# travistangvh/time-series-kafka-demo

Hardware: AMD Instinct MI355X
Metric: waveform_windows_per_sec (higher is better)
Workload: dtype bf16; 1 GPU; model=MyCNN5, global_batch=65536, seq_len=120, streams_per_gpu=65536, fs_hz=125, hipgraph=True, overlap=False, parallelism=dp1, mode=pipeline

## Files before the change

### tskd_amd/engine/stream_engine.py

```python

from __future__ import annotations

import ctypes
from typing import Optional, Sequence

import numpy as np
import os

import torch

from tskd_amd.engine import windowing as W

_plib: Optional[ctypes.CDLL] = None


def _load_preproc_lib() -> ctypes.CDLL:
    global _plib
    if _plib is not None:
        return _plib
    import os

    from tskd_amd.ops import build as _build
    path = _build.lib_path("_tskd_preprocess")
    if not os.path.exists(path):
# ... 110 lines not shown
        if chan_map is None:
            chan_map = list(range(cin))
        if self._gpu:
            lib = _load_preproc_lib()
            raw = raw.contiguous()
            is_bf16 = 1 if raw.dtype == torch.bfloat16 else 0
            if not is_bf16 and raw.dtype != torch.float32:
                raw = raw.float()
            key = tuple(chan_map)
            cm = getattr(self, "_cm_cache", {}).get(key)
            if cm is None:
                cm = torch.tensor(list(chan_map), dtype=torch.int32,
                                  device=self.device)
                self._cm_cache = getattr(self, "_cm_cache", {})
                self._cm_cache[key] = cm
            rc = lib.tskd_preproc_ingest_dense(
                ctypes.c_void_p(raw.data_ptr()), is_bf16,
                ctypes.c_void_p(self.bsum.data_ptr()),
                ctypes.c_void_p(self.bcnt.data_ptr()),
                ctypes.c_void_p(cm.data_ptr()),
                self.S, cin, self.C, t, self.G, self.bucket_len,
                ctypes.c_long(self.head), self._dstate_ptr(), self._bst,
                _sptr())
            if rc != 0:
                raise RuntimeError(f"ingest_dense failed: hipError {rc}")
            self._clear_stale_channels(chan_map, nb)
        else:
            rawf = raw.float().cpu().numpy()
            for j in range(nb):
                seg = rawf[:, :, j * self.bucket_len:(j + 1) * self.bucket_len]
                ok = ~np.isnan(seg)
                g = (self.head + j) % self.G
                for ci, c in enumerate(chan_map):
                    self.bsum[:, c, g] = torch.from_numpy(
                        np.where(ok[:, ci], seg[:, ci], 0.0).sum(-1)).float()
                    self.bcnt[:, c, g] = torch.from_numpy(
                        ok[:, ci].sum(-1).astype(np.float64)).float()
                other = [c for c in range(self.C) if c not in chan_map]
                if other:
                    self.bsum[:, other, g] = 0
                    self.bcnt[:, other, g] = 0
        self.head += nb
        self._cleared = max(self._cleared, self.head)
        self._refill()
        return nb

    def _clear_stale_channels(self, chan_map: Sequence[int], nb: int) -> None:
        other = [c for c in range(self.C) if c not in set(chan_map)]
        if not other or nb <= 0:
            return
        idx = torch.tensor([(self.head + j) % self.G for j in range(nb)],
                           dtype=torch.long, device=self.device)
        oth = torch.tensor(other, dtype=torch.long, device=self.device)
        self.bsum[:, oth[:, None], idx[None, :]] = 0
        self.bcnt[:, oth[:, None], idx[None, :]] = 0

    def ingest_events(self, stream_idx: torch.Tensor, chan_idx: torch.Tensor,
                      ts: torch.Tensor, vals: torch.Tensor,
                      advance_to: Optional[float] = None) -> None:
        if len(ts) == 0 and advance_to is None:
            return
        if (len(ts) and self.head == 0 and self.nproc == 0
                and self._origin_nproc == 0):
            first_bucket = int(float(ts.min()) // self.bucket_s)
            if first_bucket > self.G:
                self._origin_nproc = first_bucket
        min_bucket = self.nproc
        if self._gpu:
            tsd = ts.double().to(self.device) if not ts.is_cuda else ts.double()
            bucket_d = torch.floor(tsd / self.bucket_s).long()
            if len(bucket_d):
                bmax = int(bucket_d.max().item())
                bmin = int(bucket_d.min().item())
                if bmax - max(bmin, min_bucket) >= self.G - self.win_buckets:
                    raise ValueError(
                        "event batch spans more buckets than the ring "
                        "holds; ingest in smaller chunks")
                self._clear_ahead(bmax + 1)
            else:
                self._clear_ahead(0)
            lib = _load_preproc_lib()
            si = stream_idx.to(torch.int32).contiguous().to(self.device)
            ci = chan_idx.to(torch.int32).contiguous().to(self.device)
            bi = bucket_d.contiguous()
            vi = vals.float().contiguous().to(self.device)
            rc = lib.tskd_preproc_ingest_events(
                ctypes.c_void_p(si.data_ptr()), ctypes.c_void_p(ci.data_ptr()),
                ctypes.c_void_p(bi.data_ptr()), ctypes.c_void_p(vi.data_ptr()),
                ctypes.c_void_p(self.bsum.data_ptr()),
                ctypes.c_void_p(self.bcnt.data_ptr()),
                self.C, self.G, ctypes.c_long(len(vi)),
                ctypes.c_long(min_bucket), self._bst, _sptr())
            if rc != 0:
                raise RuntimeError(f"ingest_events failed: hipError {rc}")
            if advance_to is None and len(tsd):
                advance_to = float(tsd.max().item())
        else:
            bucket = torch.floor(ts.double() / self.bucket_s).long()
            if len(bucket) and int(bucket.max()) - max(int(bucket.min()),
                                                       min_bucket) \
                    >= self.G - self.win_buckets:
                raise ValueError("event batch spans more buckets than the "
                                 "ring holds; ingest in smaller chunks")
            self._clear_ahead(int(bucket.max().item()) + 1 if len(bucket)
                              else 0)
            ok = (~torch.isnan(vals)) & (bucket >= min_bucket)
            if ok.any():
                flat = ((stream_idx[ok].numpy() * self.C
                         + chan_idx[ok].numpy()) * self.G
                        + (bucket[ok].numpy() % self.G))
                bs = self.bsum.numpy().reshape(-1)
                bc = self.bcnt.numpy().reshape(-1)
                np.add.at(bs, flat, vals[ok].numpy().astype(np.float64))
                np.add.at(bc, flat, 1.0)
        hwm = float(advance_to) if advance_to is not None else float(ts.max())
        new_head = int(np.floor(hwm / self.bucket_s))
        if new_head > self.head:
            self.head = new_head
        self._refill()

    def ingest_events_chunked(self, stream_idx, chan_idx, ts, vals,
                              advance_to=None) -> None:
        cap = self.G - self.win_buckets - 1
        if len(ts) == 0:
            if advance_to is not None:
                self.ingest_events(stream_idx, chan_idx, ts, vals,
                                   advance_to=advance_to)
            return
        bucket = torch.floor(ts.double() / self.bucket_s).long()
        span = int(bucket.max()) - max(int(bucket.min()), self.nproc)
        if span < cap:
            self.ingest_events(stream_idx, chan_idx, ts, vals,
                               advance_to=advance_to)
            return
        order = torch.argsort(bucket)
        b_sorted = bucket[order]
        lo = 0
        n = len(order)
        while lo < n:
            start_bucket = max(int(b_sorted[lo]), self.nproc)
            hi = int(torch.searchsorted(b_sorted,
                                        torch.tensor(start_bucket + cap)))
            hi = max(hi, lo + 1)
            idx = order[lo:hi]
            chunk_adv = float((int(b_sorted[min(hi, n) - 1]) + 1)
                              * self.bucket_s)
            self.ingest_events(stream_idx[idx], chan_idx[idx], ts[idx],
                               vals[idx], advance_to=chunk_adv)
            lo = hi
        if advance_to is not None and advance_to / self.bucket_s > self.head:
            self._clear_ahead(int(advance_to / self.bucket_s))
            self.head = int(advance_to / self.bucket_s)
            self._refill()

    def _clear_ahead(self, upto_bucket: int) -> None:
        if upto_bucket <= self._cleared:
            return
        start = max(self._cleared, upto_bucket - self.G)
        nb = upto_bucket - start
        if self._gpu:
            lib = _load_preproc_lib()
            rc = lib.tskd_preproc_clear_buckets(
                ctypes.c_void_p(self.bsum.data_ptr()),
                ctypes.c_void_p(self.bcnt.data_ptr()),
                self.S, self.C, self.G, ctypes.c_long(start), nb,
                self._bst, _sptr())
            if rc != 0:
                raise RuntimeError(f"clear_buckets failed: hipError {rc}")
        else:
            idx = np.arange(start, start + nb) % self.G
            self.bsum[:, :, idx] = 0
            self.bcnt[:, :, idx] = 0
        self._cleared = upto_bucket

    def ingest_graph_kernel(self, raw: torch.Tensor, chan_map) -> None:
        lib = _load_preproc_lib()
        cin, t = raw.shape[1], raw.shape[2]
        key = tuple(chan_map)
        cm = getattr(self, "_cm_cache", {}).get(key)
        if cm is None:
            cm = torch.tensor(list(chan_map), dtype=torch.int32,
                              device=self.device)
            self._cm_cache = getattr(self, "_cm_cache", {})
            self._cm_cache[key] = cm
        is_bf16 = 1 if raw.dtype == torch.bfloat16 else 0
        rc = lib.tskd_preproc_ingest_dense(
            ctypes.c_void_p(raw.data_ptr()), is_bf16,
            ctypes.c_void_p(self.bsum.data_ptr()),
            ctypes.c_void_p(self.bcnt.data_ptr()),
            ctypes.c_void_p(cm.data_ptr()),
            self.S, cin, self.C, t, self.G, self.bucket_len,
            ctypes.c_long(0), self._dstate_ptr(), self._bst, _sptr())
        if rc != 0:
            raise RuntimeError(f"ingest(graph) failed: {rc}")

    def fill_graph_kernel(self, nb: int) -> None:
        lib = _load_preproc_lib()
        rc = lib.tskd_preproc_window_fill(
            ctypes.c_void_p(self.bsum.data_ptr()),
            ctypes.c_void_p(self.bcnt.data_ptr()),
            ctypes.c_void_p(self.proc.data_ptr()),
            ctypes.c_void_p(self.last_val.data_ptr()),
            self.S, self.C, self.G, ctypes.c_long(0), nb,
            self.win_buckets, self._dstate_ptr(), self._bst, _sptr())
        if rc != 0:
            raise RuntimeError(f"fill(graph) failed: {rc}")

    def ingest_dense_graph_body(self, raw: torch.Tensor, chan_map, nb: int
                                 ) -> None:
        self.ingest_graph_kernel(raw, chan_map)
        self.fill_graph_kernel(nb)

    def _refill(self) -> None:
        navail = max(0, self.head - self.win_buckets + 1)
        np_new = navail - self.nproc
        if np_new <= 0:
            return
        max_np = self.G - self.win_buckets
        if np_new > max_np:
            self.nproc = navail - max_np
            np_new = max_np
        if self._gpu:
            lib = _load_preproc_lib()
            rc = lib.tskd_preproc_window_fill(
                ctypes.c_void_p(self.bsum.data_ptr()),
                ctypes.c_void_p(self.bcnt.data_ptr()),
                ctypes.c_void_p(self.proc.data_ptr()),
                ctypes.c_void_p(self.last_val.data_ptr()),
                self.S, self.C, self.G, ctypes.c_long(self.nproc), np_new,
                self.win_buckets, self._dstate_ptr(), self._bst, _sptr())
            if rc != 0:
                raise RuntimeError(f"window_fill failed: hipError {rc}")
        else:
            bs = self.bsum.numpy()
            bc = self.bcnt.numpy()
            pr = self.proc.numpy()
            lv = self.last_val.numpy()
            span = np_new + self.win_buckets - 1
            gidx = (self.nproc + np.arange(span)) % self.G
            pidx = (self.nproc + np.arange(np_new)) % self.G
            for s in range(self.S):
                for c in range(self.C):
                    vals = W.window_averages(bs[s, c, gidx], bc[s, c, gidx],
                                             self.win_buckets)
                    filled, carry = W.fill_series(vals, lv[s, c])
                    pr[s, c, pidx] = filled
                    lv[s, c] = carry
        self.nproc = navail

    def windows(self, batch: int = 1, stride: int = 12,
                dtype: torch.dtype = torch.float32,
                out: Optional[torch.Tensor] = None,
                timelast: bool = False,
                znormalize: bool = False, zeps: float = 1e-6) -> torch.Tensor:
        B, WIN = batch, self.model_win
        assert (B - 1) * stride + WIN <= self.G, (
            f"windows(batch={B}, stride={stride}) reaches back "
            f"{(B - 1) * stride + WIN} grid points but the ring holds only "
            f"G={self.G} — older slots are already overwritten")
        shape = (self.S, B, WIN, self.C) if timelast \
            else (self.S, B, self.C, WIN)
        provided = out is not None
        if out is not None:
            assert out.shape == shape and out.dtype == dtype
            assert out.is_contiguous()
        out = out if out is not None else torch.zeros(
            shape, dtype=dtype, device=self.device)
        if self._gpu:
            lib = _load_preproc_lib()
            is_bf16 = 1 if dtype == torch.bfloat16 else 0
            assert dtype in (torch.bfloat16, torch.float32)
            rc = lib.tskd_preproc_window_gather(
                ctypes.c_void_p(self.proc.data_ptr()),
                ctypes.c_void_p(out.data_ptr()), is_bf16, int(timelast),
                self.S, self.C, self.G, B, WIN, stride,
                ctypes.c_long(self.nproc), self._dstate_ptr(),
                self._dstate_gather_extra, _sptr())
            if rc == 0 and znormalize:
                assert not timelast, "znormalize needs channel-major windows"
                rc = lib.tskd_preproc_window_znorm(
                    ctypes.c_void_p(out.data_ptr()), is_bf16,
                    ctypes.c_long(self.S * B * self.C), WIN,
                    ctypes.c_float(zeps), _sptr())
            if rc != 0:
                raise RuntimeError(f"window_gather failed: hipError {rc}")
        else:
            pr = self.proc.numpy()
            if provided:
                out.zero_()
            for b in range(B):
                wend = self.nproc - (B - 1 - b) * stride
                if wend - WIN < 0:
                    continue
                idx = (np.arange(wend - WIN, wend)) % self.G
                w = torch.from_numpy(pr[:, :, idx]).to(dtype)
                out[:, b] = w.transpose(-1, -2) if timelast else w
            if znormalize:
                assert not timelast
                m = out.float().mean(dim=-1, keepdim=True)
                sd = out.float().std(dim=-1, unbiased=False, keepdim=True)
                out.copy_(((out.float() - m) / sd.clamp_min(zeps)).to(dtype))
        return out

    @property
    def ready(self) -> bool:
        return getattr(self, "_forced_ready", False) or \
            self.nproc - self._origin_nproc >= self.model_win

    def force_ready(self) -> None:
        self._forced_ready = True


class TriggerGraph:

    def __init__(self, engine: "StreamEngine", raw: torch.Tensor,
                 chan_map, graphed_forward, stride: int = 12,
                 overlap: bool = False):
        assert engine._gpu, "TriggerGraph needs a CUDA StreamEngine"
        cin, t = raw.shape[1], raw.shape[2]
        self.nb = t // engine.bucket_len
        assert engine.nproc == engine.head - engine.win_buckets + 1, \
            "engine must be in steady state (warm up with eager triggers)"
        self.engine = engine
        self.raw = raw.contiguous()
        self.gf = graphed_forward
        self.stride = stride
        self.chan_map = list(chan_map)
        self.overlap = overlap
        dev = engine.device
        self.dstate = torch.tensor([engine.head, engine.nproc],
                                   dtype=torch.int64, device=dev)
        lib = _load_preproc_lib()
        self._lib = lib
        if overlap:
            self._init_overlap()
            return

        def trigger_body():
            engine._dstate = self.dstate
            engine._dstate_gather_extra = self.nb
            try:
                engine.ingest_dense_graph_body(self.raw, self.chan_map,
                                               self.nb)
                engine.windows(batch=1, stride=stride, dtype=self.gf.x.dtype,
                               out=self.gf.x,
                               timelast=getattr(self.gf, "timelast", False))
                out = self.gf.engine.forward(self.gf.x, self.gf.age,
                                             apply_sigmoid=True)
                rc = lib.tskd_preproc_advance_state(
                    ctypes.c_void_p(self.dstate.data_ptr()), self.nb,
                    self.nb, _sptr())
                if rc != 0:
                    raise RuntimeError(f"advance_state: {rc}")
                return out
            finally:
                engine._dstate = None
                engine._dstate_gather_extra = 0

        stream = torch.cuda.Stream()
        with torch.cuda.stream(stream):
            trigger_body()
        torch.cuda.current_stream().wait_stream(stream)
        engine.head += self.nb
        engine.nproc += self.nb
        self.graph = torch.cuda.CUDAGraph()
        with torch.cuda.graph(self.graph):
            self.out = trigger_body()

    def _init_overlap(self) -> None:
        engine, lib = self.engine, self._lib
        nb = self.nb

        def ingest_body():
            engine._dstate = self.dstate
            try:
                engine.ingest_graph_kernel(self.raw, self.chan_map)
                rc = lib.tskd_preproc_advance_state(
                    ctypes.c_void_p(self.dstate.data_ptr()), nb, 0, _sptr())
                if rc != 0:
                    raise RuntimeError(f"advance_state(head): {rc}")
            finally:
                engine._dstate = None

        def model_body():
            engine._dstate = self.dstate
            engine._dstate_gather_extra = nb
            try:
                engine.fill_graph_kernel(nb)
                engine.windows(batch=1, stride=self.stride,
                               dtype=self.gf.x.dtype, out=self.gf.x,
                               timelast=getattr(self.gf, "timelast", False))
                out = self.gf.engine.forward(self.gf.x, self.gf.age,
                                             apply_sigmoid=True)
                rc = lib.tskd_preproc_advance_state(
                    ctypes.c_void_p(self.dstate.data_ptr()), 0, nb, _sptr())
                if rc != 0:
                    raise RuntimeError(f"advance_state(nproc): {rc}")
                return out
            finally:
                engine._dstate = None
                engine._dstate_gather_extra = 0

        self._sA = torch.cuda.Stream()
        self._sB = torch.cuda.Stream()
        with torch.cuda.stream(self._sA):
            ingest_body()
        self._sB.wait_stream(self._sA)
        with torch.cuda.stream(self._sB):
            model_body()
        torch.cuda.current_stream().wait_stream(self._sB)
        engine.head += nb
        engine.nproc += nb
        self.graph_i = torch.cuda.CUDAGraph()
        with torch.cuda.graph(self.graph_i, stream=self._sA):
            ingest_body()
        self.graph_m = torch.cuda.CUDAGraph()
        with torch.cuda.graph(self.graph_m, stream=self._sB):
            self.out = model_body()
        self._evA = torch.cuda.Event()

    def replay(self, raw_refresh: bool = False) -> torch.Tensor:
        if self.overlap:
            cur = torch.cuda.current_stream()
            if raw_refresh:
                self._sA.wait_stream(cur)
            with torch.cuda.stream(self._sA):
                self.graph_i.replay()
                self._evA.record(self._sA)
            self._sB.wait_event(self._evA)
            self._sB.wait_stream(cur)
            with torch.cuda.stream(self._sB):
                self.graph_m.replay()
            cur.wait_stream(self._sB)
            self.engine.head += self.nb
            self.engine.nproc += self.nb
            return self.out
        self.graph.replay()
        self.engine.head += self.nb
        self.engine.nproc += self.nb
        return self.out
```

### tskd_amd/ops/__init__.py

```python

from __future__ import annotations

import ctypes
import os
from typing import Optional

import torch

from tskd_amd.ops import build as _build
from tskd_amd.ops.pack import (VARIANT_IDS, pack_conv1_mfma_bfrags,
                               pack_weights)

_lib: Optional[ctypes.CDLL] = None
_lib_err: Optional[str] = None


def _load_lib() -> ctypes.CDLL:
    global _lib, _lib_err
    if _lib is not None:
        return _lib
    path = _build.lib_path("_tskd_mycnn")
    if not os.path.exists(path):
        try:
            _build.build("_tskd_mycnn")
        except Exception as e:
            _lib_err = f"hipcc build failed: {e}"
            raise RuntimeError(_lib_err)
    lib = ctypes.CDLL(path)
    lib.tskd_conv_fwd.restype = ctypes.c_int
    lib.tskd_conv_fwd.argtypes = [
        ctypes.c_void_p, ctypes.c_int, ctypes.c_int, ctypes.c_void_p,
        ctypes.c_void_p, ctypes.c_void_p, ctypes.c_int, ctypes.c_int,
        ctypes.c_void_p,
    ]
    lib.tskd_debug_mfma16x16x32.restype = ctypes.c_int
    lib.tskd_debug_mfma16x16x32.argtypes = [
        ctypes.c_void_p, ctypes.c_void_p, ctypes.c_void_p, ctypes.c_void_p,
    ]
    lib.tskd_lstm_head_fwd.restype = ctypes.c_int
    lib.tskd_lstm_head_fwd.argtypes = [
        ctypes.c_void_p, ctypes.c_void_p, ctypes.c_void_p, ctypes.c_void_p,
        ctypes.c_int, ctypes.c_int, ctypes.c_float, ctypes.c_int,
        ctypes.c_int, ctypes.c_void_p,
    ]
    lib.tskd_pack_size.restype = ctypes.c_int
    lib.tskd_pack_size.argtypes = [ctypes.c_int]
    lib.tskd_feat_len.restype = ctypes.c_int
    lib.tskd_feat_len.argtypes = [ctypes.c_int]
    _lib = lib
    return lib


def hip_available() -> bool:
    try:
        _load_lib()
        return True
    except Exception:
        return False


def _stream_ptr() -> ctypes.c_void_p:
    return ctypes.c_void_p(torch.cuda.current_stream().cuda_stream)


TLAST_SLACK = 256


def alloc_windows(s: int, n: int, cin: int, win: int = 120,
                  timelast: bool = False, dtype=torch.bfloat16,
                  device="cuda") -> torch.Tensor:
    numel = s * n * cin * win
    buf = torch.zeros(numel + TLAST_SLACK, dtype=dtype, device=device)
    shape = (s, n, win, cin) if timelast else (s, n, cin, win)
    t = buf[:numel].view(*shape)
    t._tskd_slack = True
    t._tskd_buf = buf
    return t


class MyCNNEngine:

    def __init__(self, model, device: str = "cuda"):
        from tskd_amd.models.mycnn import _MyCNNBase
        assert isinstance(model, _MyCNNBase)
        self.variant = VARIANT_IDS[type(model).__name__]
        self.age_eps = float(model.AGE_EPS)
        self.cin = int(model.IN_CHANNELS)
        self.device = torch.device(device)
        self.model = model
        self.wpack = pack_weights(model).to(self.device)
        self.bfrag = pack_conv1_mfma_bfrags(model).to(self.device)
        if self.device.type == "cuda":
            lib = _load_lib()
            expect = lib.tskd_pack_size(self.variant)
            if expect != self.wpack.numel():
                raise RuntimeError(
                    f"weight pack size mismatch: py={self.wpack.numel()} "
                    f"hip={expect}")
            self.feat_len = lib.tskd_feat_len(self.variant)
        else:
            self.feat_len = int(model.MAGICNUM)

    def conv_features(self, x: torch.Tensor) -> torch.Tensor:
        timelast = (x.shape[-1] == self.cin and x.shape[-2] == 120
                    and self.cin != 120)
        lead = x.shape[:-2]
        xf = x.reshape(-1, x.shape[-2], x.shape[-1]).contiguous()
        sn = xf.shape[0]
        if xf.device.type != "cuda":
            raise RuntimeError("conv_features is the GPU path; use the model on CPU")
        lib = _load_lib()
        if timelast and (self.cin % 2 != 0 or xf.dtype != torch.bfloat16):
            xf = xf.transpose(-1, -2).contiguous()
            timelast = False
        if xf.dtype == torch.bfloat16:
            is_bf16 = 1
        elif xf.dtype == torch.float32:
            is_bf16 = 0
        else:
            xf = xf.to(torch.float32)
            is_bf16 = 0
        if timelast and not getattr(x, "_tskd_slack", False):
            pad = alloc_windows(1, sn, self.cin, 120, timelast=True,
                                dtype=xf.dtype, device=xf.device)
            pad.reshape(-1).copy_(xf.reshape(-1))
            xf = pad.reshape(sn, 120, self.cin)
        feat = torch.empty(sn, self.feat_len, dtype=torch.float32, device=xf.device)
        rc = lib.tskd_conv_fwd(
            ctypes.c_void_p(xf.data_ptr()), is_bf16, int(timelast),
            ctypes.c_void_p(feat.data_ptr()),
            ctypes.c_void_p(self.wpack.data_ptr()),
            ctypes.c_void_p(self.bfrag.data_ptr()), sn, self.variant,
            _stream_ptr())
        if rc != 0:
            raise RuntimeError(f"tskd_conv_fwd failed: hipError {rc}")
        return feat.reshape(*lead, self.feat_len)

    def lstm_head(self, feat: torch.Tensor, age: Optional[torch.Tensor],
                  apply_sigmoid: bool = False) -> torch.Tensor:
        assert feat.dim() == 3 and feat.shape[-1] == self.feat_len
        s, n = feat.shape[0], feat.shape[1]
        feat = feat.contiguous()
        lib = _load_lib()
        out = torch.empty(s, n, dtype=torch.float32, device=feat.device)
        age_ptr = ctypes.c_void_p(0)
        if age is not None:
            if age.dtype != torch.float32 or age.shape != (s, n) \
                    or not age.is_contiguous():
                age = age.to(torch.float32).expand(s, n).contiguous()
            age_ptr = ctypes.c_void_p(age.data_ptr())
        rc = lib.tskd_lstm_head_fwd(
            ctypes.c_void_p(feat.data_ptr()), age_ptr,
            ctypes.c_void_p(out.data_ptr()),
            ctypes.c_void_p(self.wpack.data_ptr()), s, n,
            ctypes.c_float(self.age_eps), int(apply_sigmoid), self.variant,
            _stream_ptr())
        if rc != 0:
            raise RuntimeError(f"tskd_lstm_head_fwd failed: hipError {rc}")
        return out

    def forward(self, x: torch.Tensor, age: Optional[torch.Tensor] = None,
                apply_sigmoid: bool = False) -> torch.Tensor:
        squeeze = x.dim() == 3
        if squeeze:
            x = x.unsqueeze(0)
            if age is not None and age.dim() == 1:
                age = age.unsqueeze(0)
        assert x.dim() == 4 and (
            (x.shape[-1] == 120 and x.shape[-2] == self.cin)
            or (x.shape[-2] == 120 and x.shape[-1] == self.cin))
        if x.device.type == "cuda":
            s, n = x.shape[0], x.shape[1]
            feat = self.conv_features(x).reshape(s, n, self.feat_len)
            out = self.lstm_head(feat, age, apply_sigmoid)
        else:
            s, n = x.shape[0], x.shape[1]
            if x.shape[-1] == self.cin and x.shape[-2] == 120:
                x = x.transpose(-1, -2)
            with torch.no_grad():
                outs = []
                for i in range(s):
                    a = age[i] if age is not None else torch.zeros(n)
                    y = self.model(x[i].float(), a.float())
                    outs.append(torch.sigmoid(y) if apply_sigmoid else y)
                out = torch.stack(outs)
        return out[0] if squeeze else out

    __call__ = forward


class GraphedForward:

    def __init__(self, engine: "MyCNNEngine", s: int, n: int,
                 dtype: torch.dtype = torch.bfloat16,
                 apply_sigmoid: bool = True, warmup: int = 2,
                 timelast: bool = False, capture: bool = True):
        assert engine.device.type == "cuda"
        self.engine = engine
        self.timelast = timelast
        self.x = alloc_windows(s, n, engine.cin, 120, timelast=timelast,
                               dtype=dtype, device=engine.device)
        self.age = torch.full((s, n), 65.0, device=engine.device)
        self.graph = None
        if not capture:
            return
        stream = torch.cuda.Stream()
        with torch.cuda.stream(stream):
            for _ in range(warmup):
                out = engine.forward(self.x, self.age,
                                     apply_sigmoid=apply_sigmoid)
        torch.cuda.current_stream().wait_stream(stream)
        self.graph = torch.cuda.CUDAGraph()
        with torch.cuda.graph(self.graph):
            self.out = engine.forward(self.x, self.age,
                                      apply_sigmoid=apply_sigmoid)

    def replay(self) -> torch.Tensor:
        self.graph.replay()
        return self.out
```

### tskd_amd/ops/csrc/mycnn_kernels.hip

```cpp

#include <hip/hip_runtime.h>
#include <stdlib.h>

#define WAVE 64
#define WG_WAVES 4
#define WG_THREADS (WAVE * WG_WAVES)

typedef __attribute__((ext_vector_type(8))) __bf16 bf16x8;
typedef __attribute__((ext_vector_type(4))) float f32x4;

template <int CIN_, int K1_, int PK_, int PS_, int L_ = 120>
struct Geom {
    static constexpr int CIN = CIN_;
    static constexpr int K1  = K1_;
    static constexpr int PK  = PK_;
    static constexpr int PS  = PS_;
    static constexpr int L   = L_;
    static constexpr int C1  = L - K1 + 1;
    static constexpr int P1  = (C1 - PK) / PS + 1;
    static constexpr int C2  = P1 - 5 + 1;
    static constexpr int LIN = (C2 - PK) / PS + 1;
    static constexpr int KK     = CIN * K1;
    static constexpr int KSTEPS = (KK + 31) / 32;
    static constexpr int MTILES = (C1 + 15) / 16;
// ... 231 lines not shown
    constexpr int NW = 4 * G::CIN * G::K1 + 4 + 20 + 1;
    __shared__ float lds_w[NW];
    __shared__ float lds_c1[WG_WAVES][4 * G::C1];
    __shared__ float lds_p1[WG_WAVES][4 * G::P1];
    __shared__ float lds_c2[WG_WAVES][G::C2];

    for (int i = threadIdx.x; i < NW; i += WG_THREADS) lds_w[i] = wpack[i];
    __syncthreads();

    const int wave = threadIdx.x / WAVE;
    const int lane = threadIdx.x % WAVE;
    const float* b1 = lds_w + G::OB1;

    bf16x8 bfr[G::KSTEPS];
    union BU { unsigned int d[4]; unsigned short u[8]; bf16x8 v; };
    #pragma unroll
    for (int st = 0; st < G::KSTEPS; ++st) {
        BU bu;
        #pragma unroll
        for (int q = 0; q < 4; ++q)
            bu.d[q] = ((const unsigned int*)bfrag)[(st * WAVE + lane) * 4 + q];
        bfr[st] = bu.v;
    }
    const int lane_dw = ((lane & 15) * G::CIN + (lane >> 4) * 8) / 2;
    __shared__ float lds_c1b[WG_WAVES][4 * G::C1];

    for (long win = (blockIdx.x * WG_WAVES + wave) * 2; win < SN;
         win += (long)gridDim.x * WG_WAVES * 2) {
        const long win1 = win + 1;
        const bool has1 = win1 < SN;
        const unsigned int* xwa =
            (const unsigned int*)(x + win * (long)(G::L * G::CIN));
        const unsigned int* xwb =
            (const unsigned int*)(x + (has1 ? win1 : win) *
                                  (long)(G::L * G::CIN));
        #pragma unroll 1
        for (int mt = 0; mt < G::MTILES; ++mt) {
            f32x4 acca = {0.f, 0.f, 0.f, 0.f};
            f32x4 accb = {0.f, 0.f, 0.f, 0.f};
            const unsigned int* basea = xwa + (long)mt * (16 * G::CIN / 2)
                                        + lane_dw;
            const unsigned int* baseb = xwb + (long)mt * (16 * G::CIN / 2)
                                        + lane_dw;
            #pragma unroll
            for (int st = 0; st < G::KSTEPS; ++st) {
                BU aa, ab;
                aa.d[0] = basea[st * 16 + 0];
                aa.d[1] = basea[st * 16 + 1];
                aa.d[2] = basea[st * 16 + 2];
                aa.d[3] = basea[st * 16 + 3];
                ab.d[0] = baseb[st * 16 + 0];
                ab.d[1] = baseb[st * 16 + 1];
                ab.d[2] = baseb[st * 16 + 2];
                ab.d[3] = baseb[st * 16 + 3];
                acca = __builtin_amdgcn_mfma_f32_16x16x32_bf16(aa.v, bfr[st],
                                                               acca, 0, 0, 0);
                accb = __builtin_amdgcn_mfma_f32_16x16x32_bf16(ab.v, bfr[st],
                                                               accb, 0, 0, 0);
            }
            const int c = lane & 15;
            if (c < 4) {
                #pragma unroll
                for (int r = 0; r < 4; ++r) {
                    const int row = mt * 16 + (lane >> 4) * 4 + r;
                    if (row < G::C1) {
                        lds_c1[wave][c * G::C1 + row] = acca[r] + b1[c];
                        lds_c1b[wave][c * G::C1 + row] = accb[r] + b1[c];
                    }
                }
            }
        }
        wave_sync();
        conv_tail<G, true>(lane, lds_w, lds_c1[wave], lds_p1[wave],
                           lds_c2[wave], feat, win);
        if (has1)
            conv_tail<G, true>(lane, lds_w, lds_c1b[wave], lds_p1[wave],
                               lds_c2[wave], feat, win1);
    }
}

template <class G>
__global__ __launch_bounds__(WG_THREADS) void conv_stack_mfma_wg_kernel(
    const unsigned short* __restrict__ x,
    float* __restrict__ feat,
    const float* __restrict__ wpack,
    const unsigned short* __restrict__ bfrag,
    int SN)
{
    constexpr int NW = 4 * G::CIN * G::K1 + 4 + 20 + 1;
    __shared__ float lds_w[NW];
    __shared__ float lds_c1[4 * G::C1];
    __shared__ float lds_p1[4 * G::P1];
    __shared__ float lds_c2[G::C2];

    for (int i = threadIdx.x; i < NW; i += WG_THREADS) lds_w[i] = wpack[i];
    __syncthreads();

    const int wave = threadIdx.x / WAVE;
    const int lane = threadIdx.x % WAVE;
    const float* b1 = lds_w + G::OB1;
    const float* w2 = lds_w + G::OW2;
    const float b2 = lds_w[G::OB2];

    bf16x8 bfr[G::KSTEPS];
    union BU { unsigned int d[4]; unsigned short u[8]; bf16x8 v; };
    #pragma unroll
    for (int st = 0; st < G::KSTEPS; ++st) {
        BU bu;
        #pragma unroll
        for (int q = 0; q < 4; ++q)
            bu.d[q] = ((const unsigned int*)bfrag)[(st * WAVE + lane) * 4 + q];
        bfr[st] = bu.v;
    }
    const int lane_dw = ((lane & 15) * G::CIN + (lane >> 4) * 8) / 2;

    for (long win = blockIdx.x; win < SN; win += gridDim.x) {
        const unsigned int* xw =
            (const unsigned int*)(x + win * (long)(G::L * G::CIN));
        for (int mt = wave; mt < G::MTILES; mt += WG_WAVES) {
            f32x4 acc = {0.f, 0.f, 0.f, 0.f};
            const unsigned int* base = xw + (long)mt * (16 * G::CIN / 2)
                                       + lane_dw;
            #pragma unroll
            for (int st = 0; st < G::KSTEPS; ++st) {
                BU au;
                au.d[0] = base[st * 16 + 0];
                au.d[1] = base[st * 16 + 1];
                au.d[2] = base[st * 16 + 2];
                au.d[3] = base[st * 16 + 3];
                acc = __builtin_amdgcn_mfma_f32_16x16x32_bf16(au.v, bfr[st],
                                                              acc, 0, 0, 0);
            }
            const int c = lane & 15;
            if (c < 4) {
                #pragma unroll
                for (int r = 0; r < 4; ++r) {
                    const int row = mt * 16 + (lane >> 4) * 4 + r;
                    if (row < G::C1)
                        lds_c1[c * G::C1 + row] = acc[r] + b1[c];
                }
            }
        }
        __syncthreads();
        for (int o = threadIdx.x; o < 4 * G::P1; o += WG_THREADS) {
            const int c = o / G::P1, q = o % G::P1;
            const float* src = lds_c1 + c * G::C1 + q * G::PS;
            float m = src[0];
            #pragma unroll
            for (int k = 1; k < G::PK; ++k) m = fmaxf(m, src[k]);
            lds_p1[o] = tanhf_(m);
        }
        __syncthreads();
        for (int s = threadIdx.x; s < G::C2; s += WG_THREADS) {
            float acc = b2;
            #pragma unroll
            for (int c = 0; c < 4; ++c) {
                const float* pr = lds_p1 + c * G::P1 + s;
                #pragma unroll
                for (int k = 0; k < 5; ++k)
                    acc = fmaf(w2[c * 5 + k], pr[k], acc);
            }
            lds_c2[s] = acc;
        }
        __syncthreads();
        for (int q = threadIdx.x; q < G::LIN; q += WG_THREADS) {
            const float* src = lds_c2 + q * G::PS;
            float m = src[0];
            #pragma unroll
            for (int k = 1; k < G::PK; ++k) m = fmaxf(m, src[k]);
            feat[win * G::LIN + q] = tanhf_(m);
        }
        __syncthreads();
    }
}

template <class G, int CHUNK = 32>
__global__ __launch_bounds__(WG_THREADS) void lstm_head_kernel(
    const float* __restrict__ feat,
    const float* __restrict__ age,
    float* __restrict__ out,
    const float* __restrict__ wpack,
    int S, int N, float age_eps, int apply_sigmoid)
{
    constexpr int LIN = G::LIN;
    constexpr int PRE_R = (CHUNK * LIN + WAVE - 1) / WAVE;
    __shared__ float lds_feat[WG_WAVES][CHUNK * LIN];

    const int wave = threadIdx.x / WAVE;
    const int lane = threadIdx.x % WAVE;
    const int unit = lane & 15;

    float wih1[LIN], whh1[16], wih2[16], whh2[16];
    const float bl1 = wpack[G::OBL1 + lane];
    const float bl2 = wpack[G::OBL2 + lane];
    #pragma unroll
    for (int i = 0; i < LIN; ++i) wih1[i] = wpack[G::OWIH1 + lane * LIN + i];
    #pragma unroll
    for (int i = 0; i < 16; ++i) {
        whh1[i] = wpack[G::OWHH1 + lane * 16 + i];
        wih2[i] = wpack[G::OWIH2 + lane * 16 + i];
        whh2[i] = wpack[G::OWHH2 + lane * 16 + i];
    }
    const float outw = wpack[G::OOUTW + unit];
    const float outb = wpack[G::OOUTB];
    const bool is_cell_gate = (lane >= 32 && lane < 48);

    float* fw = lds_feat[wave];

    for (long seq = blockIdx.x * WG_WAVES + wave; seq < S;
         seq += (long)gridDim.x * WG_WAVES) {
        const float* fseq = feat + seq * (long)N * LIN;
        const float* aseq = age ? age + seq * N : nullptr;
        float h1v[16], h2v[16];
        float c1 = 0.f, c2 = 0.f;
        #pragma unroll
        for (int u = 0; u < 16; ++u) h1v[u] = h2v[u] = 0.f;

        const long ntot = (long)N * LIN;
        float pre[PRE_R];
        #pragma unroll
        for (int r = 0; r < PRE_R; ++r) {
            const long idx = (long)r * WAVE + lane;
            pre[r] = idx < ntot ? fseq[idx] : 0.f;
        }
        for (int t0 = 0; t0 < N; t0 += CHUNK) {
            const int tn = min(CHUNK, N - t0);
            #pragma unroll
            for (int r = 0; r < PRE_R; ++r) {
                const int j = r * WAVE + lane;
                if (j < CHUNK * LIN) fw[j] = pre[r];
            }
            wave_sync();
            if (t0 + CHUNK < N) {
                const long base = (long)(t0 + CHUNK) * LIN;
                #pragma unroll
                for (int r = 0; r < PRE_R; ++r) {
                    const long idx = base + (long)r * WAVE + lane;
                    pre[r] = idx < ntot ? fseq[idx] : 0.f;
                }
            }

            for (int tt = 0; tt < tn; ++tt) {
                const float* xt = fw + tt * LIN;
                float ga = bl1, gb = 0.f;
                #pragma unroll
                for (int i = 0; i < LIN; i += 2) {
                    ga = fmaf(wih1[i], xt[i], ga);
                    if (i + 1 < LIN) gb = fmaf(wih1[i + 1], xt[i + 1], gb);
                }
                #pragma unroll
                for (int u = 0; u < 16; u += 2) {
                    ga = fmaf(whh1[u], h1v[u], ga);
                    gb = fmaf(whh1[u + 1], h1v[u + 1], gb);
                }
                float g = ga + gb;
                float a = is_cell_gate ? tanhf_(g) : sigmoidf_(g);
                {
                    const float iu = __shfl(a, unit);
                    const float fu = __shfl(a, unit + 16);
                    const float gu = __shfl(a, unit + 32);
                    const float ou = __shfl(a, unit + 48);
                    c1 = fmaf(fu, c1, iu * gu);
                    const float h = ou * tanhf_(c1);
                    #pragma unroll
                    for (int u = 0; u < 16; ++u) h1v[u] = __shfl(h, u);
                }
                ga = bl2; gb = 0.f;
                #pragma unroll
                for (int u = 0; u < 16; u += 2) {
                    ga = fmaf(wih2[u], h1v[u], ga);
                    gb = fmaf(wih2[u + 1], h1v[u + 1], gb);
                    ga = fmaf(whh2[u], h2v[u], ga);
                    gb = fmaf(whh2[u + 1], h2v[u + 1], gb);
                }
                g = ga + gb;
                a = is_cell_gate ? tanhf_(g) : sigmoidf_(g);
                {
                    const float iu = __shfl(a, unit);
                    const float fu = __shfl(a, unit + 16);
                    const float gu = __shfl(a, unit + 32);
                    const float ou = __shfl(a, unit + 48);
                    c2 = fmaf(fu, c2, iu * gu);
                    const float h = ou * tanhf_(c2);
                    #pragma unroll
                    for (int u = 0; u < 16; ++u) h2v[u] = __shfl(h, u);
                }
                if (lane == 0) {
                    float y = outb;
                    #pragma unroll
                    for (int u = 0; u < 16; ++u)
                        y = fmaf(wpack[G::OOUTW + u], h2v[u], y);
                    const float ag = aseq ? aseq[t0 + tt] : 0.f;
                    y *= fmaxf(fmaf(ag, age_eps, 1.0f), 0.0f);
                    if (apply_sigmoid) y = sigmoidf_(y);
                    out[seq * N + t0 + tt] = y;
                }
            }
            wave_sync();
        }
    }
    (void)outw;
}

__global__ void debug_mfma_kernel(const unsigned short* __restrict__ A,
                                  const unsigned short* __restrict__ B,
                                  float* __restrict__ C) {
    const int lane = threadIdx.x;
    union BU { unsigned short u[8]; bf16x8 v; } a, b;
    #pragma unroll
    for (int j = 0; j < 8; ++j) {
        const int k = (lane >> 4) * 8 + j;
        a.u[j] = A[(lane & 15) * 32 + k];
        b.u[j] = B[k * 16 + (lane & 15)];
    }
    f32x4 acc = {0.f, 0.f, 0.f, 0.f};
    acc = __builtin_amdgcn_mfma_f32_16x16x32_bf16(a.v, b.v, acc, 0, 0, 0);
    #pragma unroll
    for (int r = 0; r < 4; ++r)
        C[((lane >> 4) * 4 + r) * 16 + (lane & 15)] = acc[r];
}

namespace {

template <class G>
int launch_conv(const void* x, int x_is_bf16, int x_timelast, float* feat,
                const float* wpack, const void* bfrag, int SN,
                hipStream_t stream) {
    if (SN <= 0) return 0;
    int grid = (SN + WG_WAVES - 1) / WG_WAVES;
    if (grid > 8192) grid = 8192;
    if (x_is_bf16) {
        if (!bfrag) return -2;
        if (x_timelast) {
            if constexpr (G::CIN % 2 == 0) {
                int onewave = 1;
                if (const char* e = getenv("TSKD_CONV_TLAST_1WAVE"))
                    onewave = atoi(e);
                if (onewave) {
                    int g1 = (SN / 2 + WG_WAVES - 1) / WG_WAVES;
                    if (g1 < 1) g1 = 1;
                    if (g1 > 8192) g1 = 8192;
                    hipLaunchKernelGGL((conv_stack_mfma_tlast_kernel<G>),
                                       dim3(g1), dim3(WG_THREADS), 0, stream,
                                       (const unsigned short*)x, feat, wpack,
                                       (const unsigned short*)bfrag, SN);
                } else {
                    int g2 = SN > 16384 ? 16384 : SN;
                    hipLaunchKernelGGL((conv_stack_mfma_wg_kernel<G>),
                                       dim3(g2), dim3(WG_THREADS), 0, stream,
                                       (const unsigned short*)x, feat, wpack,
                                       (const unsigned short*)bfrag, SN);
                }
                return (int)hipGetLastError();
            }
            return -4;
        }
        hipLaunchKernelGGL((conv_stack_mfma_kernel<G>), dim3(grid),
                           dim3(WG_THREADS), 0, stream,
                           (const unsigned short*)x, feat, wpack,
                           (const unsigned short*)bfrag, SN);
    } else {
        if (x_timelast) return -4;
        hipLaunchKernelGGL((conv_stack_kernel<G>), dim3(grid),
                           dim3(WG_THREADS), 0, stream, (const float*)x, feat,
                           wpack, SN);
    }
    return (int)hipGetLastError();
}

template <class G>
int launch_lstm(const float* feat, const float* age, float* out,
                const float* wpack, int S, int N, float age_eps,
                int apply_sigmoid, hipStream_t stream) {
    if (S <= 0 || N <= 0) return 0;
    int grid = (S + WG_WAVES - 1) / WG_WAVES;
    if (grid > 8192) grid = 8192;
    int chunk = 32;
    if (const char* e = getenv("TSKD_LSTM_CHUNK")) chunk = atoi(e);
    if (chunk >= 64)
        hipLaunchKernelGGL((lstm_head_kernel<G, 64>), dim3(grid),
                           dim3(WG_THREADS), 0, stream, feat, age, out,
                           wpack, S, N, age_eps, apply_sigmoid);
    else
        hipLaunchKernelGGL((lstm_head_kernel<G, 32>), dim3(grid),
                           dim3(WG_THREADS), 0, stream, feat, age, out,
                           wpack, S, N, age_eps, apply_sigmoid);
    return (int)hipGetLastError();
}

}

extern "C" {

int tskd_conv_fwd(const void* x, int x_is_bf16, int x_timelast, float* feat,
                  const float* wpack, const void* bfrag, int SN, int variant,
                  void* stream) {
    hipStream_t s = (hipStream_t)stream;
    switch (variant) {
        case 0: return launch_conv<GeomCNN5>(x, x_is_bf16, x_timelast, feat,
                                             wpack, bfrag, SN, s);
        case 1: return launch_conv<GeomCNN2>(x, x_is_bf16, x_timelast, feat,
                                             wpack, bfrag, SN, s);
        case 2: return launch_conv<GeomCNN4>(x, x_is_bf16, x_timelast, feat,
                                             wpack, bfrag, SN, s);
    }
    return -1;
}

int tskd_lstm_head_fwd(const float* feat, const float* age, float* out,
                       const float* wpack, int S, int N, float age_eps,
                       int apply_sigmoid, int variant, void* stream) {
    hipStream_t s = (hipStream_t)stream;
    switch (variant) {
        case 0: return launch_lstm<GeomCNN5>(feat, age, out, wpack, S, N,
                                             age_eps, apply_sigmoid, s);
        case 1: return launch_lstm<GeomCNN2>(feat, age, out, wpack, S, N,
                                             age_eps, apply_sigmoid, s);
        case 2: return launch_lstm<GeomCNN4>(feat, age, out, wpack, S, N,
                                             age_eps, apply_sigmoid, s);
    }
    return -1;
}

int tskd_debug_mfma16x16x32(const unsigned short* A, const unsigned short* B,
                            float* C, void* stream) {
    hipLaunchKernelGGL(debug_mfma_kernel, dim3(1), dim3(WAVE), 0,
                       (hipStream_t)stream, A, B, C);
    return (int)hipGetLastError();
}

int tskd_pack_size(int variant) {
    switch (variant) {
        case 0: return GeomCNN5::NPACK;
        case 1: return GeomCNN2::NPACK;
        case 2: return GeomCNN4::NPACK;
    }
    return -1;
}

int tskd_feat_len(int variant) {
    switch (variant) {
        case 0: return GeomCNN5::LIN;
        case 1: return GeomCNN2::LIN;
        case 2: return GeomCNN4::LIN;
    }
    return -1;
}

int tskd_conv_ksteps(int variant) {
    switch (variant) {
        case 0: return GeomCNN5::KSTEPS;
        case 1: return GeomCNN2::KSTEPS;
        case 2: return GeomCNN4::KSTEPS;
    }
    return -1;
}

}
```

Baseline: 35.85 million windows/s.

## Fuse ring-buffer window gather, conv and LSTM head into one serve kernel

Adds a serve_tail kernel that reads the latest 120-sample window straight from the fp32 ring buffer, converts it to bf16 in LDS, and runs the MFMA conv, conv tail and LSTM head in a single launch, two windows per wave. It replaces the separate windows() gather into a bf16 staging tensor, the conv kernel writing features to global memory, and the LSTM head kernel inside the graphed trigger. This removes intermediate global round trips and kernel launches. It costs more LDS and registers per wave and only applies under the env-gated conditions of bf16, timelast, batch 1, even channel count and window 120.

```diff
diff --git a/tskd_amd/engine/stream_engine.py b/tskd_amd/engine/stream_engine.py
--- a/tskd_amd/engine/stream_engine.py
+++ b/tskd_amd/engine/stream_engine.py
@@ -436,6 +436,13 @@
                 out.copy_(((out.float() - m) / sd.clamp_min(zeps)).to(dtype))
         return out
 
+    def score_latest(self, model_engine, age: Optional[torch.Tensor] = None,
+                     apply_sigmoid: bool = True) -> torch.Tensor:
+        assert self._gpu and self.model_win == 120
+        return model_engine.score_ring(
+            self.proc, self.G, self.nproc, self._dstate_ptr(),
+            self._dstate_gather_extra, age, apply_sigmoid)
+
     @property
     def ready(self) -> bool:
         return getattr(self, "_forced_ready", False) or \
@@ -461,6 +468,13 @@
         self.stride = stride
         self.chan_map = list(chan_map)
         self.overlap = overlap
+        gf = graphed_forward
+        self.fused_tail = (
+            os.environ.get("TSKD_FUSED_TAIL", "1") != "0"
+            and gf.x.dtype == torch.bfloat16
+            and getattr(gf, "timelast", False) and gf.x.shape[1] == 1
+            and engine.model_win == 120
+            and gf.engine.supports_fused_tail(engine.C))
         dev = engine.device
         self.dstate = torch.tensor([engine.head, engine.nproc],
                                    dtype=torch.int64, device=dev)
@@ -476,11 +490,7 @@
             try:
                 engine.ingest_dense_graph_body(self.raw, self.chan_map,
                                                self.nb)
-                engine.windows(batch=1, stride=stride, dtype=self.gf.x.dtype,
-                               out=self.gf.x,
-                               timelast=getattr(self.gf, "timelast", False))
-                out = self.gf.engine.forward(self.gf.x, self.gf.age,
-                                             apply_sigmoid=True)
+                out = self._score()
                 rc = lib.tskd_preproc_advance_state(
                     ctypes.c_void_p(self.dstate.data_ptr()), self.nb,
                     self.nb, _sptr())
@@ -500,6 +510,16 @@
         self.graph = torch.cuda.CUDAGraph()
         with torch.cuda.graph(self.graph):
             self.out = trigger_body()
+
+    def _score(self) -> torch.Tensor:
+        gf = self.gf
+        if self.fused_tail:
+            return self.engine.score_latest(gf.engine, gf.age,
+                                            apply_sigmoid=True)
+        self.engine.windows(batch=1, stride=self.stride, dtype=gf.x.dtype,
+                            out=gf.x,
+                            timelast=getattr(gf, "timelast", False))
+        return gf.engine.forward(gf.x, gf.age, apply_sigmoid=True)
 
     def _init_overlap(self) -> None:
         engine, lib = self.engine, self._lib
@@ -521,11 +541,7 @@
             engine._dstate_gather_extra = nb
             try:
                 engine.fill_graph_kernel(nb)
-                engine.windows(batch=1, stride=self.stride,
-                               dtype=self.gf.x.dtype, out=self.gf.x,
-                               timelast=getattr(self.gf, "timelast", False))
-                out = self.gf.engine.forward(self.gf.x, self.gf.age,
-                                             apply_sigmoid=True)
+                out = self._score()
                 rc = lib.tskd_preproc_advance_state(
                     ctypes.c_void_p(self.dstate.data_ptr()), 0, nb, _sptr())
                 if rc != 0:
diff --git a/tskd_amd/ops/__init__.py b/tskd_amd/ops/__init__.py
--- a/tskd_amd/ops/__init__.py
+++ b/tskd_amd/ops/__init__.py
@@ -42,6 +42,13 @@
         ctypes.c_void_p, ctypes.c_void_p, ctypes.c_void_p, ctypes.c_void_p,
         ctypes.c_int, ctypes.c_int, ctypes.c_float, ctypes.c_int,
         ctypes.c_int, ctypes.c_void_p,
+    ]
+    lib.tskd_serve_tail_fwd.restype = ctypes.c_int
+    lib.tskd_serve_tail_fwd.argtypes = [
+        ctypes.c_void_p, ctypes.c_int, ctypes.c_int, ctypes.c_int,
+        ctypes.c_long, ctypes.c_void_p, ctypes.c_int, ctypes.c_void_p,
+        ctypes.c_void_p, ctypes.c_void_p, ctypes.c_void_p, ctypes.c_float,
+        ctypes.c_int, ctypes.c_int, ctypes.c_void_p,
     ]
     lib.tskd_pack_size.restype = ctypes.c_int
     lib.tskd_pack_size.argtypes = [ctypes.c_int]
@@ -159,6 +166,38 @@
             raise RuntimeError(f"tskd_lstm_head_fwd failed: hipError {rc}")
         return out
 
+    def supports_fused_tail(self, n_channels: int) -> bool:
+        return (self.device.type == "cuda" and self.cin % 2 == 0
+                and self.cin == int(n_channels))
+
+    def score_ring(self, proc: torch.Tensor, G: int, end: int,
+                   dstate_ptr=None, end_extra: int = 0,
+                   age: Optional[torch.Tensor] = None,
+                   apply_sigmoid: bool = False) -> torch.Tensor:
+        assert proc.dim() == 3 and proc.dtype == torch.float32 \
+            and proc.is_contiguous() and proc.shape[2] == G
+        s, c = proc.shape[0], proc.shape[1]
+        lib = _load_lib()
+        out = torch.empty(s, 1, dtype=torch.float32, device=proc.device)
+        age_ptr = ctypes.c_void_p(0)
+        if age is not None:
+            if age.dtype != torch.float32 or age.shape != (s, 1) \
+                    or not age.is_contiguous():
+                age = age.to(torch.float32).expand(s, 1).contiguous()
+            age_ptr = ctypes.c_void_p(age.data_ptr())
+        rc = lib.tskd_serve_tail_fwd(
+            ctypes.c_void_p(proc.data_ptr()), s, c, int(G),
+            ctypes.c_long(int(end)),
+            dstate_ptr if dstate_ptr is not None else ctypes.c_void_p(0),
+            int(end_extra), age_ptr, ctypes.c_void_p(out.data_ptr()),
+            ctypes.c_void_p(self.wpack.data_ptr()),
+            ctypes.c_void_p(self.bfrag.data_ptr()),
+            ctypes.c_float(self.age_eps), int(apply_sigmoid), self.variant,
+            _stream_ptr())
+        if rc != 0:
+            raise RuntimeError(f"tskd_serve_tail_fwd failed: code {rc}")
+        return out
+
     def forward(self, x: torch.Tensor, age: Optional[torch.Tensor] = None,
                 apply_sigmoid: bool = False) -> torch.Tensor:
         squeeze = x.dim() == 3
diff --git a/tskd_amd/ops/csrc/mycnn_kernels.hip b/tskd_amd/ops/csrc/mycnn_kernels.hip
--- a/tskd_amd/ops/csrc/mycnn_kernels.hip
+++ b/tskd_amd/ops/csrc/mycnn_kernels.hip
@@ -557,6 +557,215 @@
     (void)outw;
 }
 
+__device__ __forceinline__ unsigned int f32_to_bf16_rne(float f) {
+    union { float f; unsigned int i; } u;
+    u.f = f;
+    const unsigned int r = u.i + 0x7fffu + ((u.i >> 16) & 1);
+    return r >> 16;
+}
+
+template <class G>
+__global__ __launch_bounds__(WG_THREADS, 4) void serve_tail_kernel(
+    const float* __restrict__ proc,
+    const float* __restrict__ age,
+    float* __restrict__ out,
+    const float* __restrict__ wpack,
+    const unsigned short* __restrict__ bfrag,
+    int S, int ring, long end_in, const long long* __restrict__ dstate,
+    int end_extra, float age_eps, int apply_sigmoid)
+{
+    static_assert(G::CIN % 2 == 0, "packed staging needs an even CIN");
+    static_assert(G::XTSZ % 8 == 0 && G::XTN % 2 == 0, "");
+    constexpr int NW  = 4 * G::CIN * G::K1 + 4 + 20 + 1;
+    constexpr int LIN = G::LIN;
+    constexpr int CD  = G::CIN / 2;
+    constexpr int XTD = G::XTSZ / 2;
+    __shared__ float lds_w[NW];
+    __shared__ unsigned int lds_xt[WG_WAVES][2][XTD];
+    __shared__ float lds_c1[WG_WAVES][2][4 * G::C1];
+    static_assert(4 * G::P1 + G::C2 + LIN <= G::XTN / 2, "scratch > image");
+
+    for (int i = threadIdx.x; i < NW; i += WG_THREADS) lds_w[i] = wpack[i];
+    __syncthreads();
+
+    const int wave = __builtin_amdgcn_readfirstlane(threadIdx.x / WAVE);
+    const int lane = threadIdx.x % WAVE;
+    const int unit = lane & 15;
+    const float* b1 = lds_w + G::OB1;
+    unsigned int* xta = lds_xt[wave][0];
+    unsigned int* xtb = lds_xt[wave][1];
+    float* c1a = lds_c1[wave][0];
+    float* c1b = lds_c1[wave][1];
+    float* p1w = (float*)xta;
+    float* c2w = p1w + 4 * G::P1;
+    float* fw = c2w + G::C2;
+
+    bf16x8 bfr[G::KSTEPS];
+    union BU { unsigned int d[4]; unsigned short u[8]; bf16x8 v; };
+    #pragma unroll
+    for (int st = 0; st < G::KSTEPS; ++st) {
+        BU bu;
+        #pragma unroll
+        for (int q = 0; q < 4; ++q)
+            bu.d[q] = ((const unsigned int*)bfrag)[(st * WAVE + lane) * 4 + q];
+        bfr[st] = bu.v;
+    }
+    float wih1[LIN], wih2[16], outw[16];
+    const float bl1 = wpack[G::OBL1 + lane];
+    const float bl2 = wpack[G::OBL2 + lane];
+    #pragma unroll
+    for (int i = 0; i < LIN; ++i) wih1[i] = wpack[G::OWIH1 + lane * LIN + i];
+    #pragma unroll
+    for (int i = 0; i < 16; ++i) {
+        wih2[i] = wpack[G::OWIH2 + lane * 16 + i];
+        outw[i] = wpack[G::OOUTW + i];
+    }
+    const float outb = wpack[G::OOUTB];
+    const bool is_cell_gate = (lane >= 32 && lane < 48);
+
+    const long end = dstate ? (long)dstate[1] + end_extra : end_in;
+    const bool full = end >= G::L;
+    const int start = full ? (int)((end - G::L) % ring) : 0;
+
+    for (int i = G::XTN / 2 + lane; i < XTD; i += WAVE) xta[i] = xtb[i] = 0u;
+
+    constexpr int NT = (G::L + WAVE - 1) / WAVE;
+    unsigned int goff[NT];
+    #pragma unroll
+    for (int h = 0; h < NT; ++h) {
+        unsigned int gi = start + lane + h * WAVE;
+        if (gi >= (unsigned int)ring) gi -= ring;
+        goff[h] = gi * 4u;
+    }
+
+    auto stage = [&](unsigned int* xt, long s, bool live) {
+        const char* pr = (const char*)(proc + s * ((long)G::CIN * ring));
+        float v[NT][G::CIN];
+        #pragma unroll
+        for (int h = 0; h < NT; ++h) {
+            #pragma unroll
+            for (int c = 0; c < G::CIN; ++c) v[h][c] = 0.f;
+        }
+        if (live) {
+            #pragma unroll
+            for (int h = 0; h < NT; ++h) {
+                if (lane + h * WAVE < G::L) {
+                    #pragma unroll
+                    for (int c = 0; c < G::CIN; ++c)
+                        v[h][c] = *(const float*)(pr + (long)c * ring * 4
+                                                  + goff[h]);
+                }
+            }
+        }
+        #pragma unroll
+        for (int h = 0; h < NT; ++h) {
+            if (lane + h * WAVE < G::L) {
+                #pragma unroll
+                for (int c = 0; c < G::CIN; c += 2)
+                    xt[(lane + h * WAVE) * CD + (c >> 1)] =
+                        f32_to_bf16_rne(v[h][c]) |
+                        (f32_to_bf16_rne(v[h][c + 1]) << 16);
+            }
+        }
+    };
+
+    auto c1_store = [&](float* c1w, const f32x4& acc, int mt) {
+        const int c = lane & 15;
+        if (c < 4) {
+            #pragma unroll
+            for (int r = 0; r < 4; ++r) {
+                const int row = mt * 16 + (lane >> 4) * 4 + r;
+                if (row < G::C1) c1w[c * G::C1 + row] = acc[r] + b1[c];
+            }
+        }
+    };
+
+    auto lstm_step = [&](long s) {
+        float h1v[16], h2v[16];
+        float ga = bl1, gb = 0.f;
+        #pragma unroll
+        for (int i = 0; i < LIN; i += 2) {
+            ga = fmaf(wih1[i], fw[i], ga);
+            if (i + 1 < LIN) gb = fmaf(wih1[i + 1], fw[i + 1], gb);
+        }
+        float g = ga + gb;
+        float a = is_cell_gate ? tanhf_(g) : sigmoidf_(g);
+        {
+            const float iu = __shfl(a, unit);
+            const float gu = __shfl(a, unit + 32);
+            const float ou = __shfl(a, unit + 48);
+            const float h = ou * tanhf_(iu * gu);
+            #pragma unroll
+            for (int u = 0; u < 16; ++u) h1v[u] = __shfl(h, u);
+        }
+        ga = bl2; gb = 0.f;
+        #pragma unroll
+        for (int u = 0; u < 16; u += 2) {
+            ga = fmaf(wih2[u], h1v[u], ga);
+            gb = fmaf(wih2[u + 1], h1v[u + 1], gb);
+        }
+        g = ga + gb;
+        a = is_cell_gate ? tanhf_(g) : sigmoidf_(g);
+        {
+            const float iu = __shfl(a, unit);
+            const float gu = __shfl(a, unit + 32);
+            const float ou = __shfl(a, unit + 48);
+            const float h = ou * tanhf_(iu * gu);
+            #pragma unroll
+            for (int u = 0; u < 16; ++u) h2v[u] = __shfl(h, u);
+        }
+        if (lane == 0) {
+            float y = outb;
+            #pragma unroll
+            for (int u = 0; u < 16; ++u) y = fmaf(outw[u], h2v[u], y);
+            const float ag = age ? age[s] : 0.f;
+            y *= fmaxf(fmaf(ag, age_eps, 1.0f), 0.0f);
+            if (apply_sigmoid) y = sigmoidf_(y);
+            out[s] = y;
+        }
+        wave_sync();
+    };
+
+    for (long win = (blockIdx.x * WG_WAVES + wave) * 2; win < S;
+         win += (long)gridDim.x * WG_WAVES * 2) {
+        const long win1 = win + 1;
+        const bool has1 = win1 < S;
+        stage(xta, win, full);
+        stage(xtb, has1 ? win1 : win, full && has1);
+        wave_sync();
+
+        #pragma unroll 1
+        for (int mt = 0; mt < G::MTILES; ++mt) {
+            f32x4 acca = {0.f, 0.f, 0.f, 0.f};
+            f32x4 accb = {0.f, 0.f, 0.f, 0.f};
+            #pragma unroll
+            for (int st = 0; st < G::KSTEPS; ++st) {
+                const int bd = ((mt * 16 + (lane & 15)) * G::CIN + st * 32
+                                + (lane >> 4) * 8) / 2;
+                BU aa, ab;
+                #pragma unroll
+                for (int q = 0; q < 4; ++q) {
+                    aa.d[q] = xta[bd + q];
+                    ab.d[q] = xtb[bd + q];
+                }
+                acca = __builtin_amdgcn_mfma_f32_16x16x32_bf16(
+                    aa.v, bfr[st], acca, 0, 0, 0);
+                accb = __builtin_amdgcn_mfma_f32_16x16x32_bf16(
+                    ab.v, bfr[st], accb, 0, 0, 0);
+            }
+            c1_store(c1a, acca, mt);
+            c1_store(c1b, accb, mt);
+        }
+        wave_sync();
+        conv_tail<G, true>(lane, lds_w, c1a, p1w, c2w, fw, 0);
+        lstm_step(win);
+        if (has1) {
+            conv_tail<G, true>(lane, lds_w, c1b, p1w, c2w, fw, 0);
+            lstm_step(win1);
+        }
+    }
+}
+
 __global__ void debug_mfma_kernel(const unsigned short* __restrict__ A,
                                   const unsigned short* __restrict__ B,
                                   float* __restrict__ C) {
@@ -643,9 +852,55 @@
     return (int)hipGetLastError();
 }
 
+#define SERVE_TAIL_UNSUPPORTED (-6)
+template <class G>
+int launch_serve_tail(const float* proc, int S, int C, int ring, long end_in,
+                      const long long* dstate, int end_extra,
+                      const float* age, float* out, const float* wpack,
+                      const void* bfrag, float age_eps, int apply_sigmoid,
+                      hipStream_t stream) {
+    if constexpr (G::CIN % 2 != 0) {
+        return SERVE_TAIL_UNSUPPORTED;
+    } else {
+        if (C != G::CIN) return SERVE_TAIL_UNSUPPORTED;
+        if (ring < G::L || ring > (1 << 29)) return -5;
+        if (!bfrag) return -2;
+        if (S <= 0) return 0;
+        int g1 = (S / 2 + WG_WAVES - 1) / WG_WAVES;
+        if (g1 < 1) g1 = 1;
+        if (g1 > 8192) g1 = 8192;
+        hipLaunchKernelGGL((serve_tail_kernel<G>), dim3(g1),
+                           dim3(WG_THREADS), 0, stream, proc, age, out, wpack,
+                           (const unsigned short*)bfrag, S, ring, end_in,
+                           dstate, end_extra, age_eps, apply_sigmoid);
+        return (int)hipGetLastError();
+    }
+}
+
 }
 
 extern "C" {
+
+int tskd_serve_tail_fwd(const float* proc, int S, int C, int G, long end_in,
+                        const long long* dstate, int end_extra,
+                        const float* age, float* out, const float* wpack,
+                        const void* bfrag, float age_eps, int apply_sigmoid,
+                        int variant, void* stream) {
+    hipStream_t s = (hipStream_t)stream;
+    switch (variant) {
+        case 0: return launch_serve_tail<GeomCNN5>(
+                    proc, S, C, G, end_in, dstate, end_extra, age, out, wpack,
+                    bfrag, age_eps, apply_sigmoid, s);
+        case 1: return launch_serve_tail<GeomCNN2>(
+                    proc, S, C, G, end_in, dstate, end_extra, age, out, wpack,
+                    bfrag, age_eps, apply_sigmoid, s);
+        case 2: return launch_serve_tail<GeomCNN4>(
+                    proc, S, C, G, end_in, dstate, end_extra, age, out, wpack,
+                    bfrag, age_eps, apply_sigmoid, s);
+    }
+    return -1;
+}
+
 
 int tskd_conv_fwd(const void* x, int x_is_bf16, int x_timelast, float* feat,
                   const float* wpack, const void* bfrag, int SN, int variant,
```

New measurement: 40.69 million windows/s (median of 6 runs). 13.5% higher.
